# igd-geo/adhoc-queries-pointclouds

Measured on AMD Instinct MI355X. Metric: Mpoints/s filtered + achieved HBM GB/s, ca13 XL bounds query, 1/2/4/8 GPUs, higher is better.
Workload: dtype i32; 1 GPU; synth-ca13: 16 LAST files x 163000000 points (2608 Mpoints), query --bounds ca13_XL count-only, positions resident in HBM; points=2608000000, query=ca13_XL, launch=one batched launch per query, device=AMD Radeon Graphics gfx950:sramecc+:xnack-

## Files before the change

adhoc-queries-pointclouds_amd/csrc/chunk_index.hip:

```cpp
#include <new>

#include "pcq_internal.h"
#include "scan_tiles.h"

namespace {

constexpr int WAVES = 4;
constexpr int CHUNK_TILES = 16;
constexpr uint64_t CHUNK_POINTS = (uint64_t)CHUNK_TILES * TILE_POINTS;
constexpr uint64_t CLASS_CHUNK = 65536;


struct ChunkBox {
    int32_t mn[3], mx[3];
};

__device__ __forceinline__ int wave_min(int v) {
#pragma unroll
    for (int off = 32; off > 0; off >>= 1) v = min(v, __shfl_xor(v, off, 64));
    return v;
}
__device__ __forceinline__ int wave_max(int v) {
#pragma unroll
    for (int off = 32; off > 0; off >>= 1) v = max(v, __shfl_xor(v, off, 64));
    return v;
}

__global__ __launch_bounds__(BLOCK) void k_index_build_bounds(const v4i *__restrict__ base, uint64_t nchunks, DevPred pred,
                                                              ChunkBox *__restrict__ boxes, uint64_t *__restrict__ partials) {
    __shared__ int s_mn[WAVES][3], s_mx[WAVES][3];
    __shared__ uint64_t s_cnt[WAVES];
    const int lane = threadIdx.x & 63, wave = threadIdx.x >> 6;
    const LaneBox lb = rotate_box(pred.lo, pred.width, lane);
    const int r = lane % 3;
    uint64_t total = 0;
    for (uint64_t ch = blockIdx.x; ch < nchunks; ch += gridDim.x) {
        int mn[3] = {INT32_MAX, INT32_MAX, INT32_MAX}, mx[3] = {INT32_MIN, INT32_MIN, INT32_MIN};
#pragma unroll
        for (int q = 0; q < CHUNK_TILES / WAVES; q++) {
            const v4i *tile = base + (ch * CHUNK_TILES + (uint64_t)wave * (CHUNK_TILES / WAVES) + q) * 192;
            v4i v[3];
            v[0] = ld_nt(tile + lane);
            v[1] = ld_nt(tile + 64 + lane);
            v[2] = ld_nt(tile + 128 + lane);
            if (!pred.empty) total += tile_count_regs(v, lb);
#pragma unroll
            for (int k = 0; k < 3; k++)
#pragma unroll
                for (int j = 0; j < 4; j++) {
                    const int t = (k + j) % 3;
                    mn[t] = min(mn[t], v[k][j]);
                    mx[t] = max(mx[t], v[k][j]);
                }
        }
        int amn[3], amx[3];
#pragma unroll
        for (int c = 0; c < 3; c++) {
            const int t = (c - r + 3) % 3;
            amn[c] = t == 0 ? mn[0] : (t == 1 ? mn[1] : mn[2]);
            amx[c] = t == 0 ? mx[0] : (t == 1 ? mx[1] : mx[2]);
        }
#pragma unroll
        for (int c = 0; c < 3; c++) {
            const int a = wave_min(amn[c]), b = wave_max(amx[c]);
            if (lane == 0) s_mn[wave][c] = a, s_mx[wave][c] = b;
        }
        __syncthreads();
        if (threadIdx.x < 3) {
            const int c = threadIdx.x;
            int a = s_mn[0][c], b = s_mx[0][c];
            for (int w = 1; w < WAVES; w++) a = min(a, s_mn[w][c]), b = max(b, s_mx[w][c]);
            boxes[ch].mn[c] = a;
            boxes[ch].mx[c] = b;
        }
        __syncthreads();
    }
    if (lane == 0) s_cnt[wave] = total;
    __syncthreads();
    if (threadIdx.x == 0) partials[blockIdx.x] = s_cnt[0] + s_cnt[1] + s_cnt[2] + s_cnt[3];
}

__device__ __forceinline__ void chunk_stats_out(uint32_t n_skip, uint32_t n_full, uint32_t n_scan, unsigned long long *__restrict__ stats) {
    if (n_skip) atomicAdd(&stats[0], (unsigned long long)n_skip);
    if (n_full) atomicAdd(&stats[1], (unsigned long long)n_full);
    if (n_scan) atomicAdd(&stats[2], (unsigned long long)n_scan);
}

__global__ __launch_bounds__(BLOCK) void k_index_count_bounds(const v4i *__restrict__ base, uint64_t nchunks, DevPred pred,
                                                              const ChunkBox *__restrict__ boxes, uint64_t *__restrict__ partials,
                                                              unsigned long long *__restrict__ stats) {
    __shared__ uint64_t s_cnt[WAVES];
    const int lane = threadIdx.x & 63, wave = threadIdx.x >> 6;
    const LaneBox lb = rotate_box(pred.lo, pred.width, lane);
    int64_t hi[3];
#pragma unroll
    for (int a = 0; a < 3; a++) hi[a] = (int64_t)pred.lo[a] + (int64_t)pred.width[a];
    uint64_t total = 0;
    uint32_t n_skip = 0, n_full = 0, n_scan = 0;
    for (uint64_t ch = blockIdx.x; ch < nchunks; ch += gridDim.x) {
        const ChunkBox cb = boxes[ch];
        bool disjoint = pred.empty != 0, inside = !pred.empty;
#pragma unroll
        for (int a = 0; a < 3; a++) {
            disjoint |= (int64_t)cb.mx[a] < (int64_t)pred.lo[a] || (int64_t)cb.mn[a] > hi[a];
            inside &= (int64_t)cb.mn[a] >= (int64_t)pred.lo[a] && (int64_t)cb.mx[a] <= hi[a];
        }
        if (disjoint) {
            n_skip++;
            continue;
        }
        if (inside) {
            if (threadIdx.x == 0) total += CHUNK_POINTS;
            n_full++;
            continue;
        }
        n_scan++;
#pragma unroll
        for (int q = 0; q < CHUNK_TILES / WAVES; q++) {
            const v4i *tile = base + (ch * CHUNK_TILES + (uint64_t)wave * (CHUNK_TILES / WAVES) + q) * 192;
            v4i v[3];
            v[0] = ld_nt(tile + lane);
            v[1] = ld_nt(tile + 64 + lane);
            v[2] = ld_nt(tile + 128 + lane);
            const uint32_t c = tile_count_regs(v, lb);
            if (lane == 0) total += c;
        }
    }
    if (lane == 0) s_cnt[wave] = total;
    __syncthreads();
    if (threadIdx.x == 0) {
        partials[blockIdx.x] = s_cnt[0] + s_cnt[1] + s_cnt[2] + s_cnt[3];
        chunk_stats_out(n_skip, n_full, n_scan, stats);
    }
}

__global__ __launch_bounds__(BLOCK) void k_index_count_bounds_class(const v4i *__restrict__ base, const uint8_t *__restrict__ cls, uint64_t n,
                                                                    uint64_t nchunks, DevPred pred, const ChunkBox *__restrict__ boxes,
                                                                    const uint32_t *__restrict__ hist, uint64_t *__restrict__ partials,
                                                                    unsigned long long *__restrict__ stats) {
    __shared__ uint64_t s_cnt[WAVES];
    const int lane = threadIdx.x & 63, wave = threadIdx.x >> 6;
    const LaneBox lb = rotate_box(pred.lo, pred.width, lane);
    const Col2<COL_U8> c2 = col2_setup(cls, pred, lane, IntC<COL_U8>{});
    uint64_t total = 0;
    uint32_t n_skip = 0, n_full = 0, n_scan = 0;
    for (uint64_t ch = blockIdx.x; ch < nchunks; ch += gridDim.x) {
        const ChunkBox cb = boxes[ch];
        const uint64_t cch = ch / (CLASS_CHUNK / CHUNK_POINTS), first = cch * CLASS_CHUNK;
        const int st = index_combined_state(index_box_state(cb.mn, cb.mx, pred),
                                            index_class_state(hist[cch * 256 + (pred.cls & 255u)], n - first < CLASS_CHUNK ? n - first : CLASS_CHUNK));
        if (st == CHUNK_NONE) {
            n_skip++;
            continue;
        }
        if (st == CHUNK_ALL) {
            if (threadIdx.x == 0) total += CHUNK_POINTS;
            n_full++;
            continue;
        }
        n_scan++;
#pragma unroll
        for (int q = 0; q < CHUNK_TILES / WAVES; q++) {
            const uint64_t t = ch * CHUNK_TILES + (uint64_t)wave * (CHUNK_TILES / WAVES) + q;
            const v4i *tile = base + t * 192;
            v4i v[3];
            v[0] = ld_nt(tile + lane);
            v[1] = ld_nt(tile + 64 + lane);
            v[2] = ld_nt(tile + 128 + lane);
            Col2Regs<COL_U8> r;
            col2_load_plain(r, c2, t);
            const uint32_t c = tile_count_regs<COL_U8>(v, lb, c2, verdict_word(r, c2));
            if (lane == 0) total += c;
        }
    }
    if (lane == 0) s_cnt[wave] = total;
    __syncthreads();
    if (threadIdx.x == 0) {
        partials[blockIdx.x] = s_cnt[0] + s_cnt[1] + s_cnt[2] + s_cnt[3];
        chunk_stats_out(n_skip, n_full, n_scan, stats);
    }
}

__global__ __launch_bounds__(BLOCK) void k_index_count_bounds_time(const v4i *__restrict__ base, const uint8_t *__restrict__ times, uint64_t nchunks,
                                                                   DevPred pred, const ChunkBox *__restrict__ boxes,
                                                                   const ChunkTime *__restrict__ recs, uint64_t *__restrict__ partials,
                                                                   unsigned long long *__restrict__ stats) {
    __shared__ uint64_t s_cnt[WAVES];
    const int lane = threadIdx.x & 63, wave = threadIdx.x >> 6;
    const LaneBox lb = rotate_box(pred.lo, pred.width, lane);
    const Col2<COL_F64> c2 = col2_setup(times, pred, lane, IntC<COL_F64>{});
    uint64_t total = 0;
    uint32_t n_skip = 0, n_full = 0, n_scan = 0;
    for (uint64_t ch = blockIdx.x; ch < nchunks; ch += gridDim.x) {
        const ChunkBox cb = boxes[ch];
        const int st = index_combined_state(index_box_state(cb.mn, cb.mx, pred), index_time_state(recs[ch], c2.t0, c2.t1));
        if (st == CHUNK_NONE) {
            n_skip++;
            continue;
        }
        if (st == CHUNK_ALL) {
            if (threadIdx.x == 0) total += CHUNK_POINTS;
            n_full++;
            continue;
        }
        n_scan++;
#pragma unroll
        for (int q = 0; q < CHUNK_TILES / WAVES; q++) {
            const uint64_t t = ch * CHUNK_TILES + (uint64_t)wave * (CHUNK_TILES / WAVES) + q;
            const v4i *tile = base + t * 192;
            v4i v[3];
            v[0] = ld_nt(tile + lane);
            v[1] = ld_nt(tile + 64 + lane);
            v[2] = ld_nt(tile + 128 + lane);
            Col2Regs<COL_F64> r;
            col2_load_plain(r, c2, t);
            const uint32_t c = tile_count_regs<COL_F64>(v, lb, c2, verdict_word(r, c2));
            if (lane == 0) total += c;
        }
    }
    if (lane == 0) s_cnt[wave] = total;
    __syncthreads();
    if (threadIdx.x == 0) {
        partials[blockIdx.x] = s_cnt[0] + s_cnt[1] + s_cnt[2] + s_cnt[3];
        chunk_stats_out(n_skip, n_full, n_scan, stats);
    }
}

__global__ __launch_bounds__(BLOCK) void k_index_build_class(const uint8_t *__restrict__ cls, uint64_t n, uint64_t nchunks,
                                                             uint32_t *__restrict__ hist) {
    __shared__ uint32_t s_h[256];
    for (uint64_t ch = blockIdx.x; ch < nchunks; ch += gridDim.x) {
        s_h[threadIdx.x] = 0;
        __syncthreads();
        const uint64_t first = ch * CLASS_CHUNK;
        const uint64_t cnt = n - first < CLASS_CHUNK ? n - first : CLASS_CHUNK;
        for (uint64_t i = threadIdx.x; i < cnt; i += BLOCK) atomicAdd(&s_h[cls[first + i]], 1u);
        __syncthreads();
        hist[ch * 256 + threadIdx.x] = s_h[threadIdx.x];
        __syncthreads();
    }
}

__global__ __launch_bounds__(BLOCK) void k_index_count_class(const uint32_t *__restrict__ hist, uint64_t nchunks, uint32_t cls,
                                                             uint64_t *__restrict__ d_count) {
    __shared__ uint64_t s[BLOCK];
    uint64_t t = 0;
    for (uint64_t ch = threadIdx.x; ch < nchunks; ch += BLOCK) t += hist[ch * 256 + cls];
    s[threadIdx.x] = t;
    __syncthreads();
    for (int off = BLOCK / 2; off > 0; off >>= 1) {
        if ((int)threadIdx.x < off) s[threadIdx.x] += s[threadIdx.x + off];
        __syncthreads();
    }
    if (threadIdx.x == 0) atomicAdd((unsigned long long *)d_count, (unsigned long long)s[0]);
}

constexpr int TIME_LOADS = (int)(CHUNK_POINTS / 2 / BLOCK);
static_assert(TIME_LOADS * 2 * BLOCK == (int)CHUNK_POINTS, "a block reads a time chunk in whole loads");

__device__ __forceinline__ void load_time_chunk(v4i (&v)[TIME_LOADS], const v4i *__restrict__ base, uint64_t ch) {
    const v4i *p = base + ch * (CHUNK_POINTS / 2) + threadIdx.x;
#pragma unroll
    for (int k = 0; k < TIME_LOADS; k++) v[k] = ld_nt(p + k * BLOCK);
}
__device__ __forceinline__ uint32_t count_time_chunk(const v4i (&v)[TIME_LOADS], double t0, double t1) {
    uint32_t c = 0;
#pragma unroll
    for (int k = 0; k < TIME_LOADS; k++) c += (uint32_t)t_in(v[k][0], v[k][1], t0, t1) + (uint32_t)t_in(v[k][2], v[k][3], t0, t1);
    return c;
}
__device__ __forceinline__ void block_count_out(uint32_t cnt, uint64_t whole, uint64_t *__restrict__ partials) {
    __shared__ uint64_t s_cnt[WAVES];
    uint64_t t = cnt;
#pragma unroll
    for (int off = 32; off > 0; off >>= 1) t += __shfl_xor((unsigned long long)t, off, 64);
    if ((threadIdx.x & 63) == 0) s_cnt[threadIdx.x >> 6] = t;
    __syncthreads();
    if (threadIdx.x == 0) partials[blockIdx.x] = s_cnt[0] + s_cnt[1] + s_cnt[2] + s_cnt[3] + whole;
}

__global__ __launch_bounds__(BLOCK) void k_index_build_time(const v4i *__restrict__ base, uint64_t nchunks, DevPred pred,
                                                            ChunkTime *__restrict__ recs, uint64_t *__restrict__ partials) {
    __shared__ double s_mn[WAVES], s_mx[WAVES];
    __shared__ uint32_t s_nan[WAVES];
    const int lane = threadIdx.x & 63, wave = threadIdx.x >> 6;
    const double t0 = pred.wmin[0], t1 = pred.wmax[0];
    uint32_t cnt = 0;
    for (uint64_t ch = blockIdx.x; ch < nchunks; ch += gridDim.x) {
        v4i v[TIME_LOADS];
        load_time_chunk(v, base, ch);
        if (!pred.empty) cnt += count_time_chunk(v, t0, t1);
        double mn = __longlong_as_double(0x7ff0000000000000ll), mx = -mn;
        uint32_t nans = 0;
#pragma unroll
        for (int k = 0; k < TIME_LOADS; k++)
#pragma unroll
            for (int h = 0; h < 2; h++) {
                const double t = time_of(v[k][2 * h], v[k][2 * h + 1]);
                mn = t < mn ? t : mn;
                mx = t > mx ? t : mx;
                nans += t != t;
            }
#pragma unroll
        for (int off = 32; off > 0; off >>= 1) {
            const double a = __shfl_xor(mn, off, 64), b = __shfl_xor(mx, off, 64);
            mn = a < mn ? a : mn;
            mx = b > mx ? b : mx;
            nans += __shfl_xor(nans, off, 64);
        }
        if (lane == 0) s_mn[wave] = mn, s_mx[wave] = mx, s_nan[wave] = nans;
        __syncthreads();
        if (threadIdx.x == 0) {
            ChunkTime ct;
            ct.mn = s_mn[0], ct.mx = s_mx[0], ct.nans = s_nan[0], ct._pad = 0;
            for (int w = 1; w < WAVES; w++) {
                ct.mn = s_mn[w] < ct.mn ? s_mn[w] : ct.mn;
                ct.mx = s_mx[w] > ct.mx ? s_mx[w] : ct.mx;
                ct.nans += s_nan[w];
            }
            recs[ch] = ct;
        }
        __syncthreads();
    }
    block_count_out(cnt, 0, partials);
}

__global__ __launch_bounds__(BLOCK) void k_index_count_time(const v4i *__restrict__ base, uint64_t nchunks, DevPred pred,
                                                            const ChunkTime *__restrict__ recs, uint64_t *__restrict__ partials,
                                                            unsigned long long *__restrict__ stats) {
    const double t0 = pred.wmin[0], t1 = pred.wmax[0];
    uint32_t cnt = 0;
    uint64_t whole = 0;
    uint32_t n_skip = 0, n_full = 0, n_scan = 0;
    for (uint64_t ch = blockIdx.x; ch < nchunks; ch += gridDim.x) {
        const int st = index_time_state(recs[ch], t0, t1);
        if (st == CHUNK_NONE) {
            n_skip++;
            continue;
        }
        if (st == CHUNK_ALL) {
            whole += CHUNK_POINTS;
            n_full++;
            continue;
        }
        n_scan++;
        v4i v[TIME_LOADS];
        load_time_chunk(v, base, ch);
        cnt += count_time_chunk(v, t0, t1);
    }
    block_count_out(cnt, whole, partials);
    if (threadIdx.x == 0) chunk_stats_out(n_skip, n_full, n_scan, stats);
}

__global__ __launch_bounds__(BLOCK) void k_index_emit_stats(const ChunkBox *__restrict__ boxes, const uint32_t *__restrict__ hist,
                                                            const ChunkTime *__restrict__ times, uint64_t nchunks, uint64_t n, DevPred pred,
                                                            unsigned long long *__restrict__ stats) {
    uint32_t k[3] = {0, 0, 0};
    for (uint64_t ch = (uint64_t)blockIdx.x * BLOCK + threadIdx.x; ch < nchunks; ch += (uint64_t)gridDim.x * BLOCK) {
        int st;
        if (boxes) {
            const ChunkBox cb = boxes[ch];
            st = index_box_state(cb.mn, cb.mx, pred);
            if (hist) {
                const uint64_t cch = ch / (CLASS_CHUNK / CHUNK_POINTS), first = cch * CLASS_CHUNK;
                st = index_combined_state(st, index_class_state(hist[cch * 256 + (pred.cls & 255u)], n - first < CLASS_CHUNK ? n - first : CLASS_CHUNK));
            } else if (times) {
                st = index_combined_state(st, index_time_state(times[ch], pred.wmin[0], pred.wmax[0]));
            }
        } else if (times) {
            st = index_time_state(times[ch], pred.wmin[0], pred.wmax[0]);
        } else {
            const uint64_t first = ch * CLASS_CHUNK;
            st = index_class_state(hist[ch * 256 + (pred.cls & 255u)], n - first < CLASS_CHUNK ? n - first : CLASS_CHUNK);
        }
        k[0] += st == CHUNK_NONE, k[1] += st == CHUNK_ALL, k[2] += st == CHUNK_SCAN;
    }
#pragma unroll
    for (int a = 0; a < 3; a++) {
        uint32_t v = k[a];
#pragma unroll
        for (int off = 32; off > 0; off >>= 1) v += __shfl_xor(v, off, 64);
        if ((threadIdx.x & 63) == 0 && v) atomicAdd(&stats[a], (unsigned long long)v);
    }
}

}
static_assert(sizeof(ChunkBox) == 6 * sizeof(int32_t) && CHUNK_POINTS == INDEX_BOUNDS_CHUNK && CLASS_CHUNK == INDEX_CLASS_CHUNK,
              "EmitIndex reads the boxes as {mn[3], mx[3]}");

struct IndexPart {
    const void *col = nullptr;
    uint64_t n = 0, chunks = 0;
    void *d = nullptr;
};
struct PartRecords {
    const ChunkBox *boxes;
    const uint32_t *hist;
    const ChunkTime *times;
};

struct pcq_index {
    pcq_ctx *ctx = nullptr;
    IndexPart part[INDEX_PARTS];
    unsigned long long *d_stats = nullptr;
    pcq_index_stats last = {};
    hipStream_t stats_stream = nullptr;
    int stats_parts = 0;
    DevPred stats_pred = {};
};

static PartRecords part_records(const pcq_index *ix, int mask) {
    const void *d[INDEX_PARTS];
    for (int p = 0; p < INDEX_PARTS; p++) d[p] = (mask & INDEX_PART_BITS[p]) ? ix->part[p].d : nullptr;
    return {(const ChunkBox *)d[index_part_slot(PART_BOXES)], (const uint32_t *)d[index_part_slot(PART_HIST)],
            (const ChunkTime *)d[index_part_slot(PART_TIMES)]};
}

extern "C" int pcq_index_new(pcq_ctx *ctx, pcq_index **out) {
    PCQ_ON_DEVICE_OF_CTX(ctx);
    if (!ctx || !out) return pcq_fail(PCQ_ERR_ARG, "pcq_index_new: null argument");
    *out = nullptr;
    pcq_index *ix = new (std::nothrow) pcq_index();
    if (!ix) return pcq_fail(PCQ_ERR_NOMEM, "pcq_index_new: out of memory");
    ix->ctx = ctx;
    hipError_t e = hipMalloc((void **)&ix->d_stats, 4 * sizeof(unsigned long long));
    if (e != hipSuccess) {
        delete ix;
        return pcq_fail(PCQ_ERR_HIP, "pcq_index_new: %s", hipGetErrorString(e));
    }
    *out = ix;
    return PCQ_OK;
}

extern "C" int pcq_index_free(pcq_index *ix) {
    if (!ix) return PCQ_OK;
    PCQ_ON_DEVICE_OF_CTX(ix->ctx);
    (void)hipDeviceSynchronize();
    for (IndexPart &p : ix->part)
        if (p.d) (void)hipFree(p.d);
    if (ix->d_stats) (void)hipFree(ix->d_stats);
    delete ix;
    return PCQ_OK;
}

extern "C" int pcq_index_get_stats(pcq_index *ix, pcq_index_stats *out) {
    if (!ix || !out) return pcq_fail(PCQ_ERR_ARG, "pcq_index_get_stats: null argument");
    PCQ_ON_DEVICE_OF_CTX(ix->ctx);
    if (ix->stats_stream) {
        unsigned long long h[3] = {0, 0, 0};
        if (ix->stats_parts) {
            const uint64_t nch = ix->last.chunks, blocks = (nch + BLOCK - 1) / BLOCK;
            const int grid = (int)(blocks < (uint64_t)ix->ctx->num_cus ? blocks : (uint64_t)ix->ctx->num_cus);
            const PartRecords r = part_records(ix, ix->stats_parts);
            PCQ_HIP(hipMemsetAsync(ix->d_stats, 0, 4 * sizeof(unsigned long long), ix->stats_stream));
            if (grid > 0)
                hipLaunchKernelGGL(k_index_emit_stats, dim3(grid), dim3(BLOCK), 0, ix->stats_stream, r.boxes, r.hist, r.times, nch,
                                   ix->part[index_part_slot(PART_HIST)].n, ix->stats_pred, ix->d_stats);
            PCQ_HIP(hipGetLastError());
        }
        PCQ_HIP(hipStreamSynchronize(ix->stats_stream));
        PCQ_HIP(hipMemcpy(h, ix->d_stats, sizeof h, hipMemcpyDeviceToHost));
        ix->last.skipped = h[0];
        ix->last.whole = h[1];
        ix->last.scanned = h[2];
        ix->stats_stream = nullptr;
    }
    *out = ix->last;
    return PCQ_OK;
}

static int ensure_part(pcq_ctx *ctx, pcq_index *ix, int which, const pcq_columns *cols, uint64_t chunks, int grid, const DevPred &build_with,
                       hipStream_t s, bool *had) {
    IndexPart &p = ix->part[index_part_slot(which)];
    const void *col = index_part_column(which, *cols);
    *had = p.d && p.col == col && p.n == cols->n;
    if (*had) return PCQ_OK;
    if (p.d) PCQ_HIP(hipFree(p.d));
    p.d = nullptr;
    const size_t record = which == PART_BOXES ? sizeof(ChunkBox) : (which == PART_HIST ? 256 * sizeof(uint32_t) : sizeof(ChunkTime));
    PCQ_HIP(hipMalloc(&p.d, chunks * record));
    switch (which) {
    case PART_BOXES:
        hipLaunchKernelGGL(k_index_build_bounds, dim3(grid), dim3(BLOCK), 0, s, reinterpret_cast<const v4i *>(col), chunks, build_with, (ChunkBox *)p.d,
                           ctx->d_partials);
        break;
    case PART_HIST:
        hipLaunchKernelGGL(k_index_build_class, dim3(grid), dim3(BLOCK), 0, s, (const uint8_t *)col, cols->n, chunks, (uint32_t *)p.d);
        break;
    default:
        hipLaunchKernelGGL(k_index_build_time, dim3(grid), dim3(BLOCK), 0, s, reinterpret_cast<const v4i *>(col), chunks, build_with, (ChunkTime *)p.d,
                           ctx->d_partials);
    }
    PCQ_HIP(hipGetLastError());
    p.col = col;
    p.n = cols->n;
    p.chunks = chunks;
    return PCQ_OK;
}

static int indexed_scan(pcq_ctx *ctx, const pcq_columns *cols, const pcq_predicate *pred, const IndexPlan &pl, pcq_index *ix, pcq_collector *c,
                        void *stream, const char *entry) {
    if (c->kind == COLL_GRID) return pcq_fail(PCQ_ERR_ARG, "%s: count and buffer collectors only", entry);
    int rc = pcq_validate_scan(cols, pred, c);
    if (rc) return rc;
    DevPred dp = {};
    if (pl.parts) {
        rc = pcq_make_dev_pred(pred, &dp);
        if (rc) return rc;
    }
    ix->last = pcq_index_stats{};
    ix->stats_stream = nullptr;
    ix->stats_parts = 0;
    if (!index_covers(pl, *cols) || (pl.live_only && (dp.empty || !(dp.wmin[0] < dp.wmax[0])))) return pcq_scan_dev(ctx, cols, pred, c, stream);
    hipStream_t s = stream ? (hipStream_t)stream : ctx->stream;
    rc = pcq_scratch_stream(ctx, s);
    if (rc) return rc;
    const bool count = c->kind == COLL_COUNT;
    const uint64_t chunks = index_chunks(pl.unit, cols->n), max_blocks = (uint64_t)ctx->num_cus * 8;
    const int grid = (int)(chunks < max_blocks ? chunks : max_blocks);
    if (!pl.from_hist) {
        rc = pcq_ensure_partials(ctx, (size_t)grid);
        if (rc) return rc;
    }
    DevPred build_with = dp;
    if (!(count && pl.counts_on_build)) build_with.empty = 1;
    bool missing = false;
    for (int part : INDEX_PART_BITS) {
        if (!(pl.parts & part)) continue;
        const uint64_t pchunks = index_chunks(part, cols->n);
        bool had;
        rc = ensure_part(ctx, ix, part, cols, pchunks, (int)(pchunks < max_blocks ? pchunks : max_blocks), build_with, s, &had);
        if (rc) return rc;
        missing |= !had;
    }
    const bool pruned = !(pl.counts_on_build && missing);
    const PartRecords r = part_records(ix, pl.parts);
    ix->last.chunks = chunks;
    ix->last.built = missing;
    if (!pruned) ix->last.scanned = chunks;
    if (!count) {
        if (pruned) {
            ix->stats_stream = s;
            ix->stats_parts = pl.parts;
            ix->stats_pred = dp;
        }
        const EmitIndex eix = {reinterpret_cast<const int32_t *>(r.boxes), r.hist, r.times, index_covered_tiles(pl, cols->n)};
        return pcq_scan_dev_impl(ctx, cols, pred, c, s, &eix);
    }
    c->last_stream = s;
    if (pl.from_hist) {
        if (pruned) ix->last.whole = chunks;
        hipLaunchKernelGGL(k_index_count_class, dim3(1), dim3(BLOCK), 0, s, r.hist, chunks, (uint32_t)pred->cls, c->d_count);
        PCQ_HIP(hipGetLastError());
        return PCQ_OK;
    }
    if (pruned) {
        const v4i *xyz = reinterpret_cast<const v4i *>(cols->xyz);
        PCQ_HIP(hipMemsetAsync(ix->d_stats, 0, 4 * sizeof(unsigned long long), s));
        switch (pl.parts) {
        case PART_BOXES:
            hipLaunchKernelGGL(k_index_count_bounds, dim3(grid), dim3(BLOCK), 0, s, xyz, chunks, dp, r.boxes, ctx->d_partials, ix->d_stats);
            break;
        case PART_TIMES:
            hipLaunchKernelGGL(k_index_count_time, dim3(grid), dim3(BLOCK), 0, s, reinterpret_cast<const v4i *>(cols->cls), chunks, dp, r.times,
                               ctx->d_partials, ix->d_stats);
            break;
        case PART_BOXES | PART_HIST:
            hipLaunchKernelGGL(k_index_count_bounds_class, dim3(grid), dim3(BLOCK), 0, s, xyz, (const uint8_t *)cols->cls, cols->n, chunks, dp, r.boxes,
                               r.hist, ctx->d_partials, ix->d_stats);
            break;
        default:
            hipLaunchKernelGGL(k_index_count_bounds_time, dim3(grid), dim3(BLOCK), 0, s, xyz, (const uint8_t *)cols->cls, chunks, dp, r.boxes, r.times,
                               ctx->d_partials, ix->d_stats);
        }
        ix->stats_stream = s;
    }
    rc = pcq_launch_finish_counts(ctx, 1, grid, c->d_count, s);
    if (rc) return rc;
    const uint64_t rest_first = chunks * CHUNK_POINTS;
    if (pl.tail && rest_first < cols->n) {
        const pcq_columns tail = index_tail_columns(pl, *cols, rest_first);
        return pcq_scan_dev(ctx, &tail, pred, c, stream);
    }
    return PCQ_OK;
}

extern "C" int pcq_scan_dev_indexed(pcq_ctx *ctx, const pcq_columns *cols, const pcq_predicate *pred, pcq_index *ix,
                                    pcq_collector *c, void *stream) {
    PCQ_ON_DEVICE_OF_CTX(ctx);
    if (!ctx || !cols || !pred || !ix || !c) return pcq_fail(PCQ_ERR_ARG, "pcq_scan_dev_indexed: null argument");
    const bool own = pred->kind == PCQ_PRED_BOUNDS || pred->kind == PCQ_PRED_CLASS;
    return indexed_scan(ctx, cols, pred, own ? index_plan(pred->kind) : IndexPlan{}, ix, c, stream, "pcq_scan_dev_indexed");
}

extern "C" int pcq_scan_dev_indexed_combined(pcq_ctx *ctx, const pcq_columns *cols, const pcq_predicate *pred, pcq_index *ix,
                                             pcq_collector *c, void *stream) {
    PCQ_ON_DEVICE_OF_CTX(ctx);
    if (!ctx || !cols || !pred || !ix || !c) return pcq_fail(PCQ_ERR_ARG, "pcq_scan_dev_indexed_combined: null argument");
    if (pred->kind != PCQ_PRED_BOUNDS_CLASS)
        return pcq_fail(PCQ_ERR_ARG, "pcq_scan_dev_indexed_combined: predicate kind %d (PCQ_PRED_BOUNDS_CLASS only)", pred->kind);
    return indexed_scan(ctx, cols, pred, index_plan(pred->kind), ix, c, stream, "pcq_scan_dev_indexed_combined");
}

extern "C" int pcq_scan_dev_indexed_time(pcq_ctx *ctx, const pcq_columns *cols, const pcq_predicate *pred, pcq_index *ix,
                                         pcq_collector *c, void *stream) {
    PCQ_ON_DEVICE_OF_CTX(ctx);
    if (!ctx || !cols || !pred || !ix || !c) return pcq_fail(PCQ_ERR_ARG, "pcq_scan_dev_indexed_time: null argument");
    if (pred->kind != PCQ_PRED_TIME) return pcq_fail(PCQ_ERR_ARG, "pcq_scan_dev_indexed_time: predicate kind %d (PCQ_PRED_TIME only)", pred->kind);
    return indexed_scan(ctx, cols, pred, index_plan(pred->kind), ix, c, stream, "pcq_scan_dev_indexed_time");
}

extern "C" int pcq_scan_dev_indexed_bounds_time(pcq_ctx *ctx, const pcq_columns *cols, const pcq_predicate *pred, pcq_index *ix,
                                                pcq_collector *c, void *stream) {
    PCQ_ON_DEVICE_OF_CTX(ctx);
    if (!ctx || !cols || !pred || !ix || !c) return pcq_fail(PCQ_ERR_ARG, "pcq_scan_dev_indexed_bounds_time: null argument");
    if (pred->kind != PCQ_PRED_BOUNDS_TIME)
        return pcq_fail(PCQ_ERR_ARG, "pcq_scan_dev_indexed_bounds_time: predicate kind %d (PCQ_PRED_BOUNDS_TIME only)", pred->kind);
    return indexed_scan(ctx, cols, pred, index_plan(pred->kind), ix, c, stream, "pcq_scan_dev_indexed_bounds_time");
}
```

Measured before the change: 588,700 Mpoints/s.

## Rewrite chunk index kernels as single-wave software-pipelined streams

Replaces the four-wave-per-block chunk index build and count kernels with one-wave blocks. Each wave walks whole chunks through a double-buffered register pipeline that issues the next step's loads before evaluating the current step. Chunk records are read with scalar loads, and per-kernel waves-per-CU grid sizing replaces the fixed eight blocks per CU. The aim is to overlap HBM latency with compute in the pruned bounds count and to remove LDS reductions and __syncthreads. The cost is more register pressure, and fewer resident waves if the grid sizing is wrong.

Result: no change. 588,200 Mpoints/s (median of 3 runs) (-0.1%).

```diff
diff --git a/adhoc-queries-pointclouds_amd/csrc/chunk_index.hip b/adhoc-queries-pointclouds_amd/csrc/chunk_index.hip
--- a/adhoc-queries-pointclouds_amd/csrc/chunk_index.hip
+++ b/adhoc-queries-pointclouds_amd/csrc/chunk_index.hip
@@ -1,3 +1,5 @@
+#include <cstdio>
+#include <cstdlib>
 #include <new>
 
 #include "pcq_internal.h"
@@ -5,10 +7,20 @@
 
 namespace {
 
-constexpr int WAVES = 4;
 constexpr int CHUNK_TILES = 16;
 constexpr uint64_t CHUNK_POINTS = (uint64_t)CHUNK_TILES * TILE_POINTS;
 constexpr uint64_t CLASS_CHUNK = 65536;
+constexpr int TIME_LOADS = 4;
+constexpr uint64_t TIME_STEP_VEC = 64 * TIME_LOADS;
+constexpr uint64_t TIME_CHUNK_STEPS = CHUNK_POINTS / 2 / TIME_STEP_VEC;
+static_assert(TIME_CHUNK_STEPS * TIME_STEP_VEC * 2 == CHUNK_POINTS, "a wave reads a time chunk in whole steps");
+constexpr int INDEX_XYZ_WAVES_PER_CU = K1_WAVES_PER_CU;
+constexpr int INDEX_XYZ_COL2_WAVES_PER_CU = 4;
+constexpr int INDEX_TIME_WAVES_PER_CU = K2_WAVES_PER_CU;
+constexpr int INDEX_BUILD_XYZ_WAVES_PER_CU = 4;
+constexpr int INDEX_BUILD_TIME_WAVES_PER_CU = 6;
+constexpr int INDEX_CLASS_BLOCKS_PER_CU = 8;
+constexpr uint64_t NO_STEP = ~0ull;
 
 
 struct ChunkBox {
@@ -26,58 +38,110 @@
     return v;
 }
 
-__global__ __launch_bounds__(BLOCK) void k_index_build_bounds(const v4i *__restrict__ base, uint64_t nchunks, DevPred pred,
-                                                              ChunkBox *__restrict__ boxes, uint64_t *__restrict__ partials) {
-    __shared__ int s_mn[WAVES][3], s_mx[WAVES][3];
-    __shared__ uint64_t s_cnt[WAVES];
-    const int lane = threadIdx.x & 63, wave = threadIdx.x >> 6;
-    const LaneBox lb = rotate_box(pred.lo, pred.width, lane);
-    const int r = lane % 3;
+__device__ __forceinline__ LaneBox lane_box(const DevPred &pred, int lane) {
+    int32_t lo[3];
+    uint32_t w[3];
+#pragma unroll
+    for (int k = 0; k < 3; k++) {
+        lo[k] = pred.lo[k];
+        w[k] = pred.width[k];
+        asm volatile("" : "+s"(lo[k]), "+s"(w[k]));
+    }
+    return rotate_box(lo, w, lane);
+}
+
+template <class S, uint64_t STEPS>
+struct ChunkPipe {
+    static_assert(STEPS % 2 == 0, "every chunk starts on register set A");
+    typedef typename S::Regs Regs;
+    static constexpr int LOADS = Regs::LOADS;
+    S &s;
+    Regs A, B;
+    uint64_t pending = NO_STEP;
+    __device__ __forceinline__ explicit ChunkPipe(S &stream) : s(stream) {}
+    __device__ __forceinline__ void run(uint64_t behind) {
+#pragma nounroll
+        for (uint64_t k = 0; k < STEPS; k += 2) {
+            const uint64_t u = pending + k;
+            s.load(B, u + 1);
+            pipe_wait<LOADS>(A);
+            s.eval(A, u);
+            s.load(A, k + 2 < STEPS ? u + 2 : (behind != NO_STEP ? behind : u + 1));
+            pipe_wait<LOADS>(B);
+            s.eval(B, u + 1);
+        }
+    }
+    __device__ __forceinline__ void chunk(uint64_t ch) {
+        const uint64_t first = ch * STEPS;
+        if (pending == NO_STEP) s.load(A, first);
+        else run(first);
+        pending = first;
+    }
+    __device__ __forceinline__ void finish() {
+        if (pending == NO_STEP) return;
+        run(NO_STEP);
+        pipe_wait<0>(A);
+        pipe_wait<0>(B);
+    }
+};
+
+__device__ __forceinline__ uint32_t time_step_count(const VecRegs<TIME_LOADS> &R, double t0, double t1) {
+    uint32_t c = 0;
+#pragma unroll
+    for (int k = 0; k < TIME_LOADS; k++)
+        c += (uint32_t)__popcll(__ballot(t_in(R.r[k][0], R.r[k][1], t0, t1))) + (uint32_t)__popcll(__ballot(t_in(R.r[k][2], R.r[k][3], t0, t1)));
+    return c;
+}
+
+template <int TILES>
+struct BoxBuilder {
+    static_assert(CHUNK_TILES % TILES == 0, "a chunk is whole steps");
+    static constexpr uint64_t STEPS = CHUNK_TILES / TILES;
+    typedef PipeRegs<TILES> Regs;
+    const v4i *base;
+    ChunkBox *boxes;
+    int lane;
+    bool count;
+    LaneBox lb;
     uint64_t total = 0;
-    for (uint64_t ch = blockIdx.x; ch < nchunks; ch += gridDim.x) {
-        int mn[3] = {INT32_MAX, INT32_MAX, INT32_MAX}, mx[3] = {INT32_MIN, INT32_MIN, INT32_MIN};
-#pragma unroll
-        for (int q = 0; q < CHUNK_TILES / WAVES; q++) {
-            const v4i *tile = base + (ch * CHUNK_TILES + (uint64_t)wave * (CHUNK_TILES / WAVES) + q) * 192;
-            v4i v[3];
-            v[0] = ld_nt(tile + lane);
-            v[1] = ld_nt(tile + 64 + lane);
-            v[2] = ld_nt(tile + 128 + lane);
-            if (!pred.empty) total += tile_count_regs(v, lb);
+    int mn[3] = {INT32_MAX, INT32_MAX, INT32_MAX}, mx[3] = {INT32_MIN, INT32_MIN, INT32_MIN};
+    __device__ __forceinline__ BoxBuilder(const v4i *b, const DevPred &pred, ChunkBox *out)
+        : base(b), boxes(out), lane(threadIdx.x), count(!pred.empty), lb(lane_box(pred, threadIdx.x)) {}
+    __device__ __forceinline__ void load(Regs &R, uint64_t u) const { pipe_load<TILES>(R, base, u, lane); }
+    __device__ __forceinline__ void eval(const Regs &R, uint64_t u) {
+        if (count) total += pipe_eval<TILES>(R, lb);
+#pragma unroll
+        for (int t = 0; t < TILES; t++)
 #pragma unroll
             for (int k = 0; k < 3; k++)
 #pragma unroll
                 for (int j = 0; j < 4; j++) {
-                    const int t = (k + j) % 3;
-                    mn[t] = min(mn[t], v[k][j]);
-                    mx[t] = max(mx[t], v[k][j]);
+                    const int c = (k + j) % 3;
+                    mn[c] = min(mn[c], R.r[t][k][j]);
+                    mx[c] = max(mx[c], R.r[t][k][j]);
                 }
-        }
-        int amn[3], amx[3];
+        if ((u + 1) % STEPS != 0) return;
+        const int r = lane % 3;
+        ChunkBox cb;
 #pragma unroll
         for (int c = 0; c < 3; c++) {
             const int t = (c - r + 3) % 3;
-            amn[c] = t == 0 ? mn[0] : (t == 1 ? mn[1] : mn[2]);
-            amx[c] = t == 0 ? mx[0] : (t == 1 ? mx[1] : mx[2]);
-        }
-#pragma unroll
-        for (int c = 0; c < 3; c++) {
-            const int a = wave_min(amn[c]), b = wave_max(amx[c]);
-            if (lane == 0) s_mn[wave][c] = a, s_mx[wave][c] = b;
-        }
-        __syncthreads();
-        if (threadIdx.x < 3) {
-            const int c = threadIdx.x;
-            int a = s_mn[0][c], b = s_mx[0][c];
-            for (int w = 1; w < WAVES; w++) a = min(a, s_mn[w][c]), b = max(b, s_mx[w][c]);
-            boxes[ch].mn[c] = a;
-            boxes[ch].mx[c] = b;
-        }
-        __syncthreads();
-    }
-    if (lane == 0) s_cnt[wave] = total;
-    __syncthreads();
-    if (threadIdx.x == 0) partials[blockIdx.x] = s_cnt[0] + s_cnt[1] + s_cnt[2] + s_cnt[3];
+            cb.mn[c] = wave_min(t == 0 ? mn[0] : (t == 1 ? mn[1] : mn[2]));
+            cb.mx[c] = wave_max(t == 0 ? mx[0] : (t == 1 ? mx[1] : mx[2]));
+        }
+        if (lane == 0) boxes[u / STEPS] = cb;
+#pragma unroll
+        for (int c = 0; c < 3; c++) mn[c] = INT32_MAX, mx[c] = INT32_MIN;
+    }
+};
+template <int TILES = K1_TILES>
+__global__ __launch_bounds__(64) void k_index_build_bounds(const v4i *__restrict__ base, uint64_t nchunks, DevPred pred,
+                                                           ChunkBox *__restrict__ boxes, uint64_t *__restrict__ partials) {
+    BoxBuilder<TILES> s(base, pred, boxes);
+    ChunkPipe<BoxBuilder<TILES>, BoxBuilder<TILES>::STEPS> pipe(s);
+    for (uint64_t ch = blockIdx.x; ch < nchunks; ch += gridDim.x) pipe.chunk(ch);
+    pipe.finish();
+    if (threadIdx.x == 0) partials[blockIdx.x] = s.total;
 }
 
 __device__ __forceinline__ void chunk_stats_out(uint32_t n_skip, uint32_t n_full, uint32_t n_scan, unsigned long long *__restrict__ stats) {
@@ -86,144 +150,123 @@
     if (n_scan) atomicAdd(&stats[2], (unsigned long long)n_scan);
 }
 
-__global__ __launch_bounds__(BLOCK) void k_index_count_bounds(const v4i *__restrict__ base, uint64_t nchunks, DevPred pred,
-                                                              const ChunkBox *__restrict__ boxes, uint64_t *__restrict__ partials,
-                                                              unsigned long long *__restrict__ stats) {
-    __shared__ uint64_t s_cnt[WAVES];
-    const int lane = threadIdx.x & 63, wave = threadIdx.x >> 6;
-    const LaneBox lb = rotate_box(pred.lo, pred.width, lane);
-    int64_t hi[3];
-#pragma unroll
-    for (int a = 0; a < 3; a++) hi[a] = (int64_t)pred.lo[a] + (int64_t)pred.width[a];
+template <typename T>
+__device__ __forceinline__ T record_word(const T *p) {
+    static_assert(sizeof(T) == 4 || sizeof(T) == 8, "one or two dwords");
+    T v = *(const __attribute__((address_space(4))) T *)p;
+    asm volatile("" : "+s"(v));
+    return v;
+}
+__device__ __forceinline__ int chunk_box_state(const ChunkBox *boxes, uint64_t ch, const DevPred &pred) {
+    int32_t mn[3], mx[3];
+#pragma unroll
+    for (int k = 0; k < 3; k++) mn[k] = record_word(&boxes[ch].mn[k]), mx[k] = record_word(&boxes[ch].mx[k]);
+    return index_box_state(mn, mx, pred);
+}
+__device__ __forceinline__ int chunk_time_state(const ChunkTime *recs, uint64_t ch, double t0, double t1) {
+    ChunkTime ct;
+    ct.mn = __longlong_as_double((long long)record_word(reinterpret_cast<const uint64_t *>(&recs[ch].mn)));
+    ct.mx = __longlong_as_double((long long)record_word(reinterpret_cast<const uint64_t *>(&recs[ch].mx)));
+    ct.nans = record_word(&recs[ch].nans);
+    ct._pad = 0;
+    return index_time_state(ct, t0, t1);
+}
+template <int COL>
+struct ChunkRecs {
+    typedef char type;
+};
+template <>
+struct ChunkRecs<COL_U8> {
+    typedef uint32_t type;
+};
+template <>
+struct ChunkRecs<COL_F64> {
+    typedef ChunkTime type;
+};
+template <int COL>
+__device__ __forceinline__ int chunk_state(uint64_t ch, const DevPred &pred, const ChunkBox *boxes, const typename ChunkRecs<COL>::type *recs, uint64_t n) {
+    const int st = chunk_box_state(boxes, ch, pred);
+    if constexpr (COL == COL_U8) {
+        const uint64_t cch = ch / (CLASS_CHUNK / CHUNK_POINTS), first = cch * CLASS_CHUNK;
+        return index_combined_state(st, index_class_state(record_word(&recs[cch * 256 + (pred.cls & 255u)]), n - first < CLASS_CHUNK ? n - first : CLASS_CHUNK));
+    } else if constexpr (COL == COL_F64) {
+        return index_combined_state(st, chunk_time_state(recs, ch, pred.wmin[0], pred.wmax[0]));
+    } else {
+        return st;
+    }
+}
+
+struct ChunkWalk {
+    uint64_t whole = 0;
+    uint32_t n_skip = 0, n_full = 0, n_scan = 0;
+    __device__ __forceinline__ bool reads(int st) {
+        if (st == CHUNK_SCAN) {
+            n_scan++;
+            return true;
+        }
+        if (st == CHUNK_NONE) n_skip++;
+        else n_full++, whole += CHUNK_POINTS;
+        return false;
+    }
+};
+__device__ __forceinline__ void chunk_walk_out(uint64_t total, const ChunkWalk &w, uint64_t *__restrict__ partials, unsigned long long *__restrict__ stats) {
+    if (threadIdx.x != 0) return;
+    partials[blockIdx.x] = total + w.whole;
+    chunk_stats_out(w.n_skip, w.n_full, w.n_scan, stats);
+}
+
+template <int TILES, int COL>
+struct k_index_count_pipe {
+    static_assert(CHUNK_TILES % TILES == 0, "a chunk is whole steps");
+    static constexpr uint64_t STEPS = CHUNK_TILES / TILES;
+    typedef PipeRegs<TILES, COL> Regs;
+    const v4i *base;
+    int lane;
+    LaneBox lb;
+    Col2<COL> c2;
     uint64_t total = 0;
-    uint32_t n_skip = 0, n_full = 0, n_scan = 0;
-    for (uint64_t ch = blockIdx.x; ch < nchunks; ch += gridDim.x) {
-        const ChunkBox cb = boxes[ch];
-        bool disjoint = pred.empty != 0, inside = !pred.empty;
-#pragma unroll
-        for (int a = 0; a < 3; a++) {
-            disjoint |= (int64_t)cb.mx[a] < (int64_t)pred.lo[a] || (int64_t)cb.mn[a] > hi[a];
-            inside &= (int64_t)cb.mn[a] >= (int64_t)pred.lo[a] && (int64_t)cb.mx[a] <= hi[a];
-        }
-        if (disjoint) {
-            n_skip++;
-            continue;
-        }
-        if (inside) {
-            if (threadIdx.x == 0) total += CHUNK_POINTS;
-            n_full++;
-            continue;
-        }
-        n_scan++;
-#pragma unroll
-        for (int q = 0; q < CHUNK_TILES / WAVES; q++) {
-            const v4i *tile = base + (ch * CHUNK_TILES + (uint64_t)wave * (CHUNK_TILES / WAVES) + q) * 192;
-            v4i v[3];
-            v[0] = ld_nt(tile + lane);
-            v[1] = ld_nt(tile + 64 + lane);
-            v[2] = ld_nt(tile + 128 + lane);
-            const uint32_t c = tile_count_regs(v, lb);
-            if (lane == 0) total += c;
-        }
-    }
-    if (lane == 0) s_cnt[wave] = total;
-    __syncthreads();
-    if (threadIdx.x == 0) {
-        partials[blockIdx.x] = s_cnt[0] + s_cnt[1] + s_cnt[2] + s_cnt[3];
-        chunk_stats_out(n_skip, n_full, n_scan, stats);
-    }
-}
-
-__global__ __launch_bounds__(BLOCK) void k_index_count_bounds_class(const v4i *__restrict__ base, const uint8_t *__restrict__ cls, uint64_t n,
-                                                                    uint64_t nchunks, DevPred pred, const ChunkBox *__restrict__ boxes,
-                                                                    const uint32_t *__restrict__ hist, uint64_t *__restrict__ partials,
-                                                                    unsigned long long *__restrict__ stats) {
-    __shared__ uint64_t s_cnt[WAVES];
-    const int lane = threadIdx.x & 63, wave = threadIdx.x >> 6;
-    const LaneBox lb = rotate_box(pred.lo, pred.width, lane);
-    const Col2<COL_U8> c2 = col2_setup(cls, pred, lane, IntC<COL_U8>{});
-    uint64_t total = 0;
-    uint32_t n_skip = 0, n_full = 0, n_scan = 0;
-    for (uint64_t ch = blockIdx.x; ch < nchunks; ch += gridDim.x) {
-        const ChunkBox cb = boxes[ch];
-        const uint64_t cch = ch / (CLASS_CHUNK / CHUNK_POINTS), first = cch * CLASS_CHUNK;
-        const int st = index_combined_state(index_box_state(cb.mn, cb.mx, pred),
-                                            index_class_state(hist[cch * 256 + (pred.cls & 255u)], n - first < CLASS_CHUNK ? n - first : CLASS_CHUNK));
-        if (st == CHUNK_NONE) {
-            n_skip++;
-            continue;
-        }
-        if (st == CHUNK_ALL) {
-            if (threadIdx.x == 0) total += CHUNK_POINTS;
-            n_full++;
-            continue;
-        }
-        n_scan++;
-#pragma unroll
-        for (int q = 0; q < CHUNK_TILES / WAVES; q++) {
-            const uint64_t t = ch * CHUNK_TILES + (uint64_t)wave * (CHUNK_TILES / WAVES) + q;
-            const v4i *tile = base + t * 192;
-            v4i v[3];
-            v[0] = ld_nt(tile + lane);
-            v[1] = ld_nt(tile + 64 + lane);
-            v[2] = ld_nt(tile + 128 + lane);
-            Col2Regs<COL_U8> r;
-            col2_load_plain(r, c2, t);
-            const uint32_t c = tile_count_regs<COL_U8>(v, lb, c2, verdict_word(r, c2));
-            if (lane == 0) total += c;
-        }
-    }
-    if (lane == 0) s_cnt[wave] = total;
-    __syncthreads();
-    if (threadIdx.x == 0) {
-        partials[blockIdx.x] = s_cnt[0] + s_cnt[1] + s_cnt[2] + s_cnt[3];
-        chunk_stats_out(n_skip, n_full, n_scan, stats);
-    }
-}
-
-__global__ __launch_bounds__(BLOCK) void k_index_count_bounds_time(const v4i *__restrict__ base, const uint8_t *__restrict__ times, uint64_t nchunks,
-                                                                   DevPred pred, const ChunkBox *__restrict__ boxes,
-                                                                   const ChunkTime *__restrict__ recs, uint64_t *__restrict__ partials,
-                                                                   unsigned long long *__restrict__ stats) {
-    __shared__ uint64_t s_cnt[WAVES];
-    const int lane = threadIdx.x & 63, wave = threadIdx.x >> 6;
-    const LaneBox lb = rotate_box(pred.lo, pred.width, lane);
-    const Col2<COL_F64> c2 = col2_setup(times, pred, lane, IntC<COL_F64>{});
-    uint64_t total = 0;
-    uint32_t n_skip = 0, n_full = 0, n_scan = 0;
-    for (uint64_t ch = blockIdx.x; ch < nchunks; ch += gridDim.x) {
-        const ChunkBox cb = boxes[ch];
-        const int st = index_combined_state(index_box_state(cb.mn, cb.mx, pred), index_time_state(recs[ch], c2.t0, c2.t1));
-        if (st == CHUNK_NONE) {
-            n_skip++;
-            continue;
-        }
-        if (st == CHUNK_ALL) {
-            if (threadIdx.x == 0) total += CHUNK_POINTS;
-            n_full++;
-            continue;
-        }
-        n_scan++;
-#pragma unroll
-        for (int q = 0; q < CHUNK_TILES / WAVES; q++) {
-            const uint64_t t = ch * CHUNK_TILES + (uint64_t)wave * (CHUNK_TILES / WAVES) + q;
-            const v4i *tile = base + t * 192;
-            v4i v[3];
-            v[0] = ld_nt(tile + lane);
-            v[1] = ld_nt(tile + 64 + lane);
-            v[2] = ld_nt(tile + 128 + lane);
-            Col2Regs<COL_F64> r;
-            col2_load_plain(r, c2, t);
-            const uint32_t c = tile_count_regs<COL_F64>(v, lb, c2, verdict_word(r, c2));
-            if (lane == 0) total += c;
-        }
-    }
-    if (lane == 0) s_cnt[wave] = total;
-    __syncthreads();
-    if (threadIdx.x == 0) {
-        partials[blockIdx.x] = s_cnt[0] + s_cnt[1] + s_cnt[2] + s_cnt[3];
-        chunk_stats_out(n_skip, n_full, n_scan, stats);
-    }
+    __device__ __forceinline__ k_index_count_pipe(const v4i *b, const DevPred &pred, const uint8_t *col)
+        : base(b), lane(threadIdx.x), lb(lane_box(pred, threadIdx.x)), c2(col2_setup(col, pred, threadIdx.x, IntC<COL>{})) {}
+    __device__ __forceinline__ void load(Regs &R, uint64_t u) const { pipe_load<TILES, COL>(R, base, u, lane, c2); }
+    __device__ __forceinline__ void eval(const Regs &R, uint64_t) { total += pipe_eval<TILES, COL>(R, lb, c2); }
+};
+__global__ __launch_bounds__(64) void k_index_count_bounds(const v4i *__restrict__ base, uint64_t nchunks, DevPred pred,
+                                                           const ChunkBox *__restrict__ boxes, uint64_t *__restrict__ partials,
+                                                           unsigned long long *__restrict__ stats) {
+    typedef k_index_count_pipe<K1_TILES, COL_NONE> Stream;
+    Stream s(base, pred, nullptr);
+    ChunkPipe<Stream, Stream::STEPS> pipe(s);
+    ChunkWalk w;
+    for (uint64_t ch = blockIdx.x; ch < nchunks; ch += gridDim.x)
+        if (w.reads(chunk_state<COL_NONE>(ch, pred, boxes, nullptr, 0))) pipe.chunk(ch);
+    pipe.finish();
+    chunk_walk_out(s.total, w, partials, stats);
+}
+__global__ __launch_bounds__(64) void k_index_count_bounds_class(const v4i *__restrict__ base, const uint8_t *__restrict__ cls, uint64_t n,
+                                                                 uint64_t nchunks, DevPred pred, const ChunkBox *__restrict__ boxes,
+                                                                 const uint32_t *__restrict__ hist, uint64_t *__restrict__ partials,
+                                                                 unsigned long long *__restrict__ stats) {
+    typedef k_index_count_pipe<K1_TILES, COL_U8> Stream;
+    Stream s(base, pred, cls);
+    ChunkPipe<Stream, Stream::STEPS> pipe(s);
+    ChunkWalk w;
+    for (uint64_t ch = blockIdx.x; ch < nchunks; ch += gridDim.x)
+        if (w.reads(chunk_state<COL_U8>(ch, pred, boxes, hist, n))) pipe.chunk(ch);
+    pipe.finish();
+    chunk_walk_out(s.total, w, partials, stats);
+}
+__global__ __launch_bounds__(64) void k_index_count_bounds_time(const v4i *__restrict__ base, const uint8_t *__restrict__ times, uint64_t nchunks,
+                                                                DevPred pred, const ChunkBox *__restrict__ boxes,
+                                                                const ChunkTime *__restrict__ recs, uint64_t *__restrict__ partials,
+                                                                unsigned long long *__restrict__ stats) {
+    typedef k_index_count_pipe<K1_TILES, COL_F64> Stream;
+    Stream s(base, pred, times);
+    ChunkPipe<Stream, Stream::STEPS> pipe(s);
+    ChunkWalk w;
+    for (uint64_t ch = blockIdx.x; ch < nchunks; ch += gridDim.x)
+        if (w.reads(chunk_state<COL_F64>(ch, pred, boxes, recs, 0))) pipe.chunk(ch);
+    pipe.finish();
+    chunk_walk_out(s.total, w, partials, stats);
 }
 
 __global__ __launch_bounds__(BLOCK) void k_index_build_class(const uint8_t *__restrict__ cls, uint64_t n, uint64_t nchunks,
@@ -255,52 +298,41 @@
     if (threadIdx.x == 0) atomicAdd((unsigned long long *)d_count, (unsigned long long)s[0]);
 }
 
-constexpr int TIME_LOADS = (int)(CHUNK_POINTS / 2 / BLOCK);
-static_assert(TIME_LOADS * 2 * BLOCK == (int)CHUNK_POINTS, "a block reads a time chunk in whole loads");
-
-__device__ __forceinline__ void load_time_chunk(v4i (&v)[TIME_LOADS], const v4i *__restrict__ base, uint64_t ch) {
-    const v4i *p = base + ch * (CHUNK_POINTS / 2) + threadIdx.x;
-#pragma unroll
-    for (int k = 0; k < TIME_LOADS; k++) v[k] = ld_nt(p + k * BLOCK);
-}
-__device__ __forceinline__ uint32_t count_time_chunk(const v4i (&v)[TIME_LOADS], double t0, double t1) {
-    uint32_t c = 0;
-#pragma unroll
-    for (int k = 0; k < TIME_LOADS; k++) c += (uint32_t)t_in(v[k][0], v[k][1], t0, t1) + (uint32_t)t_in(v[k][2], v[k][3], t0, t1);
-    return c;
-}
-__device__ __forceinline__ void block_count_out(uint32_t cnt, uint64_t whole, uint64_t *__restrict__ partials) {
-    __shared__ uint64_t s_cnt[WAVES];
-    uint64_t t = cnt;
-#pragma unroll
-    for (int off = 32; off > 0; off >>= 1) t += __shfl_xor((unsigned long long)t, off, 64);
-    if ((threadIdx.x & 63) == 0) s_cnt[threadIdx.x >> 6] = t;
-    __syncthreads();
-    if (threadIdx.x == 0) partials[blockIdx.x] = s_cnt[0] + s_cnt[1] + s_cnt[2] + s_cnt[3] + whole;
-}
-
-__global__ __launch_bounds__(BLOCK) void k_index_build_time(const v4i *__restrict__ base, uint64_t nchunks, DevPred pred,
-                                                            ChunkTime *__restrict__ recs, uint64_t *__restrict__ partials) {
-    __shared__ double s_mn[WAVES], s_mx[WAVES];
-    __shared__ uint32_t s_nan[WAVES];
-    const int lane = threadIdx.x & 63, wave = threadIdx.x >> 6;
-    const double t0 = pred.wmin[0], t1 = pred.wmax[0];
-    uint32_t cnt = 0;
-    for (uint64_t ch = blockIdx.x; ch < nchunks; ch += gridDim.x) {
-        v4i v[TIME_LOADS];
-        load_time_chunk(v, base, ch);
-        if (!pred.empty) cnt += count_time_chunk(v, t0, t1);
-        double mn = __longlong_as_double(0x7ff0000000000000ll), mx = -mn;
-        uint32_t nans = 0;
+
+struct TimeStream {
+    static constexpr uint64_t STEPS = TIME_CHUNK_STEPS;
+    typedef VecRegs<TIME_LOADS> Regs;
+    const v4i *base;
+    int lane;
+    bool count;
+    double t0, t1;
+    uint64_t total = 0;
+    __device__ __forceinline__ TimeStream(const v4i *b, const DevPred &pred, bool counts)
+        : base(b), lane(threadIdx.x), count(counts), t0(pred.wmin[0]), t1(pred.wmax[0]) {}
+    __device__ __forceinline__ void load(Regs &R, uint64_t u) const { vec_load(R, base + u * TIME_STEP_VEC, lane); }
+    __device__ __forceinline__ void eval(const Regs &R, uint64_t) {
+        if (count) total += time_step_count(R, t0, t1);
+    }
+};
+struct TimeBuilder : TimeStream {
+    ChunkTime *recs;
+    double mn, mx;
+    uint32_t nans = 0;
+    __device__ __forceinline__ static double inf() { return __longlong_as_double(0x7ff0000000000000ll); }
+    __device__ __forceinline__ TimeBuilder(const v4i *b, const DevPred &pred, ChunkTime *out)
+        : TimeStream(b, pred, !pred.empty), recs(out), mn(inf()), mx(-inf()) {}
+    __device__ __forceinline__ void eval(const Regs &R, uint64_t u) {
+        TimeStream::eval(R, u);
 #pragma unroll
         for (int k = 0; k < TIME_LOADS; k++)
 #pragma unroll
             for (int h = 0; h < 2; h++) {
-                const double t = time_of(v[k][2 * h], v[k][2 * h + 1]);
+                const double t = time_of(R.r[k][2 * h], R.r[k][2 * h + 1]);
                 mn = t < mn ? t : mn;
                 mx = t > mx ? t : mx;
                 nans += t != t;
             }
+        if ((u + 1) % STEPS != 0) return;
 #pragma unroll
         for (int off = 32; off > 0; off >>= 1) {
             const double a = __shfl_xor(mn, off, 64), b = __shfl_xor(mx, off, 64);
@@ -308,48 +340,33 @@
             mx = b > mx ? b : mx;
             nans += __shfl_xor(nans, off, 64);
         }
-        if (lane == 0) s_mn[wave] = mn, s_mx[wave] = mx, s_nan[wave] = nans;
-        __syncthreads();
-        if (threadIdx.x == 0) {
+        if (lane == 0) {
             ChunkTime ct;
-            ct.mn = s_mn[0], ct.mx = s_mx[0], ct.nans = s_nan[0], ct._pad = 0;
-            for (int w = 1; w < WAVES; w++) {
-                ct.mn = s_mn[w] < ct.mn ? s_mn[w] : ct.mn;
-                ct.mx = s_mx[w] > ct.mx ? s_mx[w] : ct.mx;
-                ct.nans += s_nan[w];
-            }
-            recs[ch] = ct;
-        }
-        __syncthreads();
-    }
-    block_count_out(cnt, 0, partials);
-}
-
-__global__ __launch_bounds__(BLOCK) void k_index_count_time(const v4i *__restrict__ base, uint64_t nchunks, DevPred pred,
-                                                            const ChunkTime *__restrict__ recs, uint64_t *__restrict__ partials,
-                                                            unsigned long long *__restrict__ stats) {
-    const double t0 = pred.wmin[0], t1 = pred.wmax[0];
-    uint32_t cnt = 0;
-    uint64_t whole = 0;
-    uint32_t n_skip = 0, n_full = 0, n_scan = 0;
-    for (uint64_t ch = blockIdx.x; ch < nchunks; ch += gridDim.x) {
-        const int st = index_time_state(recs[ch], t0, t1);
-        if (st == CHUNK_NONE) {
-            n_skip++;
-            continue;
-        }
-        if (st == CHUNK_ALL) {
-            whole += CHUNK_POINTS;
-            n_full++;
-            continue;
-        }
-        n_scan++;
-        v4i v[TIME_LOADS];
-        load_time_chunk(v, base, ch);
-        cnt += count_time_chunk(v, t0, t1);
-    }
-    block_count_out(cnt, whole, partials);
-    if (threadIdx.x == 0) chunk_stats_out(n_skip, n_full, n_scan, stats);
+            ct.mn = mn, ct.mx = mx, ct.nans = nans, ct._pad = 0;
+            recs[u / STEPS] = ct;
+        }
+        mn = inf(), mx = -inf(), nans = 0;
+    }
+};
+__global__ __launch_bounds__(64) void k_index_build_time(const v4i *__restrict__ base, uint64_t nchunks, DevPred pred,
+                                                         ChunkTime *__restrict__ recs, uint64_t *__restrict__ partials) {
+    TimeBuilder s(base, pred, recs);
+    ChunkPipe<TimeBuilder, TimeBuilder::STEPS> pipe(s);
+    for (uint64_t ch = blockIdx.x; ch < nchunks; ch += gridDim.x) pipe.chunk(ch);
+    pipe.finish();
+    if (threadIdx.x == 0) partials[blockIdx.x] = s.total;
+}
+
+__global__ __launch_bounds__(64) void k_index_count_time(const v4i *__restrict__ base, uint64_t nchunks, DevPred pred,
+                                                         const ChunkTime *__restrict__ recs, uint64_t *__restrict__ partials,
+                                                         unsigned long long *__restrict__ stats) {
+    TimeStream s(base, pred, true);
+    ChunkPipe<TimeStream, TimeStream::STEPS> pipe(s);
+    ChunkWalk w;
+    for (uint64_t ch = blockIdx.x; ch < nchunks; ch += gridDim.x)
+        if (w.reads(chunk_time_state(recs, ch, s.t0, s.t1))) pipe.chunk(ch);
+    pipe.finish();
+    chunk_walk_out(s.total, w, partials, stats);
 }
 
 __global__ __launch_bounds__(BLOCK) void k_index_emit_stats(const ChunkBox *__restrict__ boxes, const uint32_t *__restrict__ hist,
@@ -469,8 +486,24 @@
     return PCQ_OK;
 }
 
-static int ensure_part(pcq_ctx *ctx, pcq_index *ix, int which, const pcq_columns *cols, uint64_t chunks, int grid, const DevPred &build_with,
-                       hipStream_t s, bool *had) {
+static int index_grid(const pcq_ctx *ctx, int parts, uint64_t chunks, bool builder) {
+    int per_cu;
+    if (builder) per_cu = parts == PART_HIST ? INDEX_CLASS_BLOCKS_PER_CU : (parts == PART_BOXES ? INDEX_BUILD_XYZ_WAVES_PER_CU : INDEX_BUILD_TIME_WAVES_PER_CU);
+    else per_cu = !(parts & PART_BOXES) ? INDEX_TIME_WAVES_PER_CU : ((parts & ~PART_BOXES) ? INDEX_XYZ_COL2_WAVES_PER_CU : INDEX_XYZ_WAVES_PER_CU);
+#ifdef PCQ_LAB
+    if (const char *e = getenv("PCQ_INDEX_W")) {
+        int w[4] = {0, 0, 0, 0};
+        sscanf(e, "%d,%d,%d,%d", &w[0], &w[1], &w[2], &w[3]);
+        const int k = ((parts & PART_BOXES) ? 0 : 1) + (builder ? 2 : 0);
+        if (!(builder && parts == PART_HIST) && w[k] > 0 && w[k] <= 8) per_cu = w[k];
+    }
+#endif
+    const uint64_t most = (uint64_t)ctx->num_cus * (uint64_t)per_cu;
+    return (int)(chunks < most ? chunks : most);
+}
+
+static int ensure_part(pcq_ctx *ctx, pcq_index *ix, int which, const pcq_columns *cols, uint64_t chunks, const DevPred &build_with, hipStream_t s,
+                       bool *had) {
     IndexPart &p = ix->part[index_part_slot(which)];
     const void *col = index_part_column(which, *cols);
     *had = p.d && p.col == col && p.n == cols->n;
@@ -479,16 +512,17 @@
     p.d = nullptr;
     const size_t record = which == PART_BOXES ? sizeof(ChunkBox) : (which == PART_HIST ? 256 * sizeof(uint32_t) : sizeof(ChunkTime));
     PCQ_HIP(hipMalloc(&p.d, chunks * record));
+    const int grid = index_grid(ctx, which, chunks, true);
     switch (which) {
     case PART_BOXES:
-        hipLaunchKernelGGL(k_index_build_bounds, dim3(grid), dim3(BLOCK), 0, s, reinterpret_cast<const v4i *>(col), chunks, build_with, (ChunkBox *)p.d,
-                           ctx->d_partials);
+        hipLaunchKernelGGL(k_index_build_bounds<K1_TILES>, dim3(grid), dim3(64), 0, s, reinterpret_cast<const v4i *>(col), chunks, build_with,
+                           (ChunkBox *)p.d, ctx->d_partials);
         break;
     case PART_HIST:
         hipLaunchKernelGGL(k_index_build_class, dim3(grid), dim3(BLOCK), 0, s, (const uint8_t *)col, cols->n, chunks, (uint32_t *)p.d);
         break;
     default:
-        hipLaunchKernelGGL(k_index_build_time, dim3(grid), dim3(BLOCK), 0, s, reinterpret_cast<const v4i *>(col), chunks, build_with, (ChunkTime *)p.d,
+        hipLaunchKernelGGL(k_index_build_time, dim3(grid), dim3(64), 0, s, reinterpret_cast<const v4i *>(col), chunks, build_with, (ChunkTime *)p.d,
                            ctx->d_partials);
     }
     PCQ_HIP(hipGetLastError());
@@ -516,10 +550,14 @@
     rc = pcq_scratch_stream(ctx, s);
     if (rc) return rc;
     const bool count = c->kind == COLL_COUNT;
-    const uint64_t chunks = index_chunks(pl.unit, cols->n), max_blocks = (uint64_t)ctx->num_cus * 8;
-    const int grid = (int)(chunks < max_blocks ? chunks : max_blocks);
+    const uint64_t chunks = index_chunks(pl.unit, cols->n);
+    const int grid = index_grid(ctx, pl.parts, chunks, false), build_grid = index_grid(ctx, pl.unit, chunks, true);
     if (!pl.from_hist) {
-        rc = pcq_ensure_partials(ctx, (size_t)grid);
+        const uint64_t max_blocks = (uint64_t)ctx->num_cus * 8;
+        static_assert(INDEX_XYZ_WAVES_PER_CU <= 8 && INDEX_XYZ_COL2_WAVES_PER_CU <= 8 && INDEX_TIME_WAVES_PER_CU <= 8 && INDEX_BUILD_XYZ_WAVES_PER_CU <= 8 &&
+                          INDEX_BUILD_TIME_WAVES_PER_CU <= 8 && INDEX_CLASS_BLOCKS_PER_CU == 8,
+                      "no grid of the index is wider than eight workgroups per CU");
+        rc = pcq_ensure_partials(ctx, (size_t)(chunks < max_blocks ? chunks : max_blocks));
         if (rc) return rc;
     }
     DevPred build_with = dp;
@@ -529,7 +567,7 @@
         if (!(pl.parts & part)) continue;
         const uint64_t pchunks = index_chunks(part, cols->n);
         bool had;
-        rc = ensure_part(ctx, ix, part, cols, pchunks, (int)(pchunks < max_blocks ? pchunks : max_blocks), build_with, s, &had);
+        rc = ensure_part(ctx, ix, part, cols, pchunks, build_with, s, &had);
         if (rc) return rc;
         missing |= !had;
     }
@@ -559,23 +597,23 @@
         PCQ_HIP(hipMemsetAsync(ix->d_stats, 0, 4 * sizeof(unsigned long long), s));
         switch (pl.parts) {
         case PART_BOXES:
-            hipLaunchKernelGGL(k_index_count_bounds, dim3(grid), dim3(BLOCK), 0, s, xyz, chunks, dp, r.boxes, ctx->d_partials, ix->d_stats);
+            hipLaunchKernelGGL(k_index_count_bounds, dim3(grid), dim3(64), 0, s, xyz, chunks, dp, r.boxes, ctx->d_partials, ix->d_stats);
             break;
         case PART_TIMES:
-            hipLaunchKernelGGL(k_index_count_time, dim3(grid), dim3(BLOCK), 0, s, reinterpret_cast<const v4i *>(cols->cls), chunks, dp, r.times,
+            hipLaunchKernelGGL(k_index_count_time, dim3(grid), dim3(64), 0, s, reinterpret_cast<const v4i *>(cols->cls), chunks, dp, r.times,
                                ctx->d_partials, ix->d_stats);
             break;
         case PART_BOXES | PART_HIST:
-            hipLaunchKernelGGL(k_index_count_bounds_class, dim3(grid), dim3(BLOCK), 0, s, xyz, (const uint8_t *)cols->cls, cols->n, chunks, dp, r.boxes,
+            hipLaunchKernelGGL(k_index_count_bounds_class, dim3(grid), dim3(64), 0, s, xyz, (const uint8_t *)cols->cls, cols->n, chunks, dp, r.boxes,
                                r.hist, ctx->d_partials, ix->d_stats);
             break;
         default:
-            hipLaunchKernelGGL(k_index_count_bounds_time, dim3(grid), dim3(BLOCK), 0, s, xyz, (const uint8_t *)cols->cls, chunks, dp, r.boxes, r.times,
+            hipLaunchKernelGGL(k_index_count_bounds_time, dim3(grid), dim3(64), 0, s, xyz, (const uint8_t *)cols->cls, chunks, dp, r.boxes, r.times,
                                ctx->d_partials, ix->d_stats);
         }
         ix->stats_stream = s;
     }
-    rc = pcq_launch_finish_counts(ctx, 1, grid, c->d_count, s);
+    rc = pcq_launch_finish_counts(ctx, 1, pruned ? grid : build_grid, c->d_count, s);
     if (rc) return rc;
     const uint64_t rest_first = chunks * CHUNK_POINTS;
     if (pl.tail && rest_first < cols->n) {
```
